# neverorfrog/vehicle-control

Hardware: AMD Instinct MI355X
Metric: MPC solves/sec (batched, N=20) (higher is better)
Workload: dtype f64; 1 GPU; C2 kinematic-bicycle LTV-MPC, B=1024 per GPU, N=20, fp64; batch_per_gpu=1024, global_batch=1024, horizon=20, parallelism=dp1 (independent shards)

## Files before the change

vehicle-control_amd/csrc/kin_ltv.hip:

```cpp
#include <hip/hip_runtime.h>

#include <cstdint>

#include "vc_kernels.hpp"
#include "vc_models.hpp"
#include "vcmpc.h"

#ifndef KIN_NU_TOL
#define KIN_NU_TOL 1e-10
#endif
#ifndef KIN_EARLY_F
#define KIN_EARLY_F 100.0
#endif
#ifndef KIN_EARLY_ROUNDS
#define KIN_EARLY_ROUNDS 2
#endif
#ifndef KIN_TAPIA_F
#define KIN_TAPIA_F 1.02
#endif
#ifndef KIN_DUAL_TOL
#define KIN_DUAL_TOL 1e-12
#endif
#ifndef KIN_AL_RHO
#define KIN_AL_RHO 1e1
#endif
#ifndef KIN_DOT_CH
#define KIN_DOT_CH 8
#endif
#ifndef KIN_UPDATE
#define KIN_UPDATE 1
#endif
#ifndef KIN_RSQ_HALLEY
#define KIN_RSQ_HALLEY 1
#endif
#ifndef KIN_STAT_CHECK
#define KIN_STAT_CHECK 0
#endif
#ifndef KIN_STEP_F
#define KIN_STEP_F 0.99
#endif
#ifndef KIN_SOLVE_CH
#define KIN_SOLVE_CH 8
#endif
#ifndef KIN_PANEL_CH
#define KIN_PANEL_CH 6
#endif

namespace vc {
namespace {

__device__ __forceinline__ double lane_bcast(double v, int src) {
  const int lo = __builtin_amdgcn_readlane(__double2loint(v), src);
  const int hi = __builtin_amdgcn_readlane(__double2hiint(v), src);
  return __hiloint2double(hi, lo);
}
__device__ int amdgcn_writelane(int v, int lane, int old) __asm("llvm.amdgcn.writelane.i32");
__device__ __forceinline__ double lane_put(double old, double v, int dst) {
  const int lo = amdgcn_writelane(__double2loint(v), dst, __double2loint(old));
  const int hi = amdgcn_writelane(__double2hiint(v), dst, __double2hiint(old));
  return __hiloint2double(hi, lo);
}
template <int K>
__device__ __forceinline__ double dpp_row_shr(double v, double ident) {
  const int lo = __builtin_amdgcn_update_dpp(__double2loint(ident), __double2loint(v), 0x110 + K, 0xf, 0xf, false);
  const int hi = __builtin_amdgcn_update_dpp(__double2hiint(ident), __double2hiint(v), 0x110 + K, 0xf, 0xf, false);
  return __hiloint2double(hi, lo);
}
template <typename Op>
__device__ __forceinline__ double wave_reduce(double v, double ident, Op op) {
  v = op(v, dpp_row_shr<1>(v, ident));
  v = op(v, dpp_row_shr<2>(v, ident));
  v = op(v, dpp_row_shr<4>(v, ident));
  v = op(v, dpp_row_shr<8>(v, ident));
  return op(op(lane_bcast(v, 15), lane_bcast(v, 31)), op(lane_bcast(v, 47), lane_bcast(v, 63)));
}
__device__ __forceinline__ double wave_sum(double v) {
  return wave_reduce(v, 0.0, [](double a, double b) { return a + b; });
}
__device__ __forceinline__ double wave_max(double v) {
  return wave_reduce(v, -__builtin_inf(), [](double a, double b) { return fmax(a, b); });
}
__device__ __forceinline__ double wave_min(double v) {
  return wave_reduce(v, __builtin_inf(), [](double a, double b) { return fmin(a, b); });
}
__device__ __forceinline__ void wave_sync() {
  asm volatile("" ::: "memory");
  __builtin_amdgcn_wave_barrier();
  asm volatile("" ::: "memory");
}
__device__ __forceinline__ void fence() { __builtin_amdgcn_sched_barrier(0); }
__device__ __forceinline__ int lane_opaque(int lane) {
  asm volatile("" : "+v"(lane));
  return lane;
}
__device__ __forceinline__ void no_hoist() { asm volatile("" ::: "memory"); }

using lds_cdouble = const __attribute__((address_space(3))) double;
__device__ __forceinline__ lds_cdouble* lds_opaque(const double* p) {
  uint32_t a = (uint32_t)(uintptr_t)(lds_cdouble*)p;
  asm volatile("" : "+v"(a));
  return (lds_cdouble*)(uintptr_t)a;
}

#ifdef VC_TIMING
#define VC_TSTAMP(var) \
  fence();              \
  const uint64_t var = __builtin_amdgcn_s_memtime(); \
  fence();
#define VC_TACC(slot, t0) \
  {                      \
    fence();             \
    tacc[slot] += __builtin_amdgcn_s_memtime() - (t0); \
    fence();             \
  }
#else
#define VC_TSTAMP(var)
#define VC_TACC(slot, t0)
#endif
enum { T_SWEEP = 0, T_SETUP, T_RESID, T_BUILD, T_CHOL, T_SOLVE, T_UPDATE, T_POLISH, T_OUT, T_S2, T_S3, T_S4, T_PAL, T_PPASS, T_NUPD, T_UCYC, T_NDROP, T_CFAIL, T_CRM, T_CADD, T_R0CHG, T_NSLOT };


template <int N>
struct Dims {
  static constexpr int n = 2 * N;
  static constexpr int NC = 2 * (N - 1);
  static constexpr int LD = n + 1;
  static_assert(n <= 64 && N >= 2, "one wavefront per problem needs 2 <= N <= 32");
};

template <int n>
__host__ __device__ constexpr int lc_base(int k) {
  static_assert(n % 2 == 0, "even n");
  return k * (n - 1) - k * (k - 1) / 2 + (k + 1) / 2;
}
template <int n>
__host__ __device__ constexpr int lc_start(int k) {
  return lc_base<n>(k) + k;
}

template <int N>
struct Smem {
  using D = Dims<N>;
  static constexpr int LC_DUMMY = lc_start<D::n>(D::n);
  static constexpr int LC_ZERO = LC_DUMMY + 1;
  double G[D::NC + 3][D::LD];
  double H[D::n + 1][D::LD];
  alignas(16) double Lc[LC_ZERO + 1];
  alignas(16) double zrow[48];
  double xb[N + 1][KIN_NX + 1];
  double jac[N + 1][9];
  double ub[D::n];
  double kap[N], ds[N];
  union {
    struct {
      double vz[64];
      double vc[64];
    };
    alignas(16) double tb2[128];
  };
  double dinv[64];
};

template <int N>
__host__ __device__ constexpr int crow_stage(int r) {
  return r < N - 1 ? r + 1 : r - (N - 1) + 1;
}

template <int LEN, int SA, int SB, int CH = KIN_DOT_CH>
__device__ __forceinline__ double lds_dot(lds_cdouble* a, lds_cdouble* b) {
  constexpr int NCH = (LEN + CH - 1) / CH;
  double ca[2][CH], cb[2][CH];
  auto fetch = [&](int c, int buf) {
#pragma unroll
    for (int q = 0; q < CH; ++q) {
      const int i = c * CH + q;
      ca[buf][q] = (i < LEN) ? a[i * SA] : 0.0;
      cb[buf][q] = (i < LEN) ? b[i * SB] : 0.0;
    }
  };
  double a0 = 0.0, a1 = 0.0;
  fetch(0, 0);
#pragma unroll
  for (int c = 0; c < NCH; ++c) {
    if (c + 1 < NCH) fetch(c + 1, (c + 1) & 1);
    fence();
#pragma unroll
    for (int q = 0; q < CH; q += 2) {
      a0 += ca[c & 1][q] * cb[c & 1][q];
      a1 += ca[c & 1][q + 1] * cb[c & 1][q + 1];
    }
  }
  fence();
  return a0 + a1;
}

template <int N>
__device__ double grow_dot(const Smem<N>& s, int lane) {
  constexpr int NC = Dims<N>::NC;
  const int r = lane < NC ? lane : 0;
  const double a = lds_dot<2 * (N - 1), 1, 1>(lds_opaque(&s.G[r][0]), lds_opaque(&s.vz[0]));
  return lane < NC ? a : 0.0;
}

template <int N>
__device__ double gt_dot(const Smem<N>& s, int lane) {
  constexpr int n = Dims<N>::n, NC = Dims<N>::NC, LD = Dims<N>::LD;
  const int j = lane < n ? lane : 0;
  const double a = lds_dot<NC, LD, 1>(lds_opaque(&s.G[0][j]), lds_opaque(&s.vc[0]));
  return lane < n ? a : 0.0;
}


template <int N>
__device__ double h_dot(const Smem<N>& s, int lane) {
  constexpr int n = Dims<N>::n;
  const int j = lane < n ? lane : 0;
  return lds_dot<n, 1, 1>(lds_opaque(&s.H[j][0]), lds_opaque(&s.vz[0]));
}

__device__ __forceinline__ void kin_sincos(double x, double& sn, double& cs) {
  const double n = __builtin_rint(x * 6.36619772367581382433e-01);
  const double y = fma(-n, 6.07710050650619224932e-11, fma(-n, 1.57079632673412561417e+00, x));
  const double z = y * y;
  const double rs = fma(z, fma(z, fma(z, fma(z, 1.58969099521155010221e-10, -2.50507602534068634195e-08),
                                      2.75573137070700676789e-06), -1.98412698298579493134e-04),
                        8.33333333332248946124e-03);
  const double sk = fma(z * y, fma(z, rs, -1.66666666666666324348e-01), y);
  const double rc = z * fma(z, fma(z, fma(z, fma(z, fma(z, -1.13596475577881948265e-11, 2.08757232129817482790e-09),
                                                  -2.75573143513906633035e-07), 2.48015872894767294178e-05),
                                   -1.38888888888741095749e-03), 4.16666666666666019037e-02);
  const double hz = 0.5 * z, w = 1.0 - hz;
  const double ck = w + (((1.0 - w) - hz) + z * rc);
  const int q = int(n) & 3;
  const double a = (q & 1) ? ck : sk, b = (q & 1) ? sk : ck;
  sn = (q & 2) ? -a : a;
  cs = ((q + 1) & 2) ? -b : b;
}

__device__ __forceinline__ double rsq_nr(double d) {
  double inv = __builtin_amdgcn_rsq(d);
#if KIN_RSQ_HALLEY
  const double e = fma(-d, inv * inv, 1.0);
  return fma(inv * e, fma(0.375, e, 0.5), inv);
#else
  inv = inv * (1.5 - 0.5 * d * inv * inv);
  inv = inv * (1.5 - 0.5 * d * inv * inv);
  return inv;
#endif
}

template <int N>
__device__ __forceinline__ void store_rows(const double (&Mr)[Dims<N>::n], Smem<N>& s, int lane) {
}

template <int N>
__device__ double chol_solve(const double (&Lr)[Dims<N>::n], const Smem<N>& s, double b, int lane) {
  constexpr int n = Dims<N>::n;
  constexpr int CH = KIN_SOLVE_CH;
  static_assert(n % CH == 0, "backward prefetch chunks");
  const int row = lane < n ? lane : 0;
  lds_cdouble* col = lds_opaque(&s.Lc[lc_base<n>(row)]);
  const double dj = s.dinv[row];
  double acc = b;
#pragma unroll
  for (int k = 0; k < n; ++k) acc -= Lr[k] * lane_bcast(acc * dj, k);
  acc *= dj;
  double x = 0.0;
  double lk[2][CH];
  lds_cdouble* zero = lds_opaque(&s.zrow[0]);
  auto fetch = [&](int c, int buf) {
    lds_cdouble* src = row < n - 1 - c * CH ? col : zero;
#pragma unroll
    for (int q = 0; q < CH; ++q) lk[buf][q] = src[n - 1 - c * CH - q];
  };
  fetch(0, 0);
#pragma unroll
  for (int c = 0; c < n / CH; ++c) {
    if (c + 1 < n / CH) fetch(c + 1, (c + 1) & 1);
    fence();
#pragma unroll
    for (int q = 0; q < CH; ++q) {
      const int k = n - 1 - c * CH - q;
      const double xk = lane_bcast(acc * dj, k);
      x = lane_put(x, xk, k);
      acc -= lk[c & 1][q] * xk;
    }
    fence();
  }
  return x;
}

enum { ROWS_G = 0, ROWS_E = 1 };
template <int N, int KIND>
__host__ __device__ constexpr int row_extent(int r) {
  if (KIND == ROWS_G) return r < Dims<N>::NC ? 2 * crow_stage<N>(r) : 0;
  return r < N ? 2 * (r + 1) : (r < N + 2 ? 2 * N : 0);
}
template <int N, int KIND>
__host__ __device__ constexpr int gram_rows() {
  return KIND == ROWS_G ? Dims<N>::NC : N + 2;
}
template <int N, int KIND>
__host__ __device__ constexpr bool kstep_hits(int ks, int I) {
  for (int q = 0; q < 4; ++q)
    if (row_extent<N, KIND>(4 * ks + q) > 16 * I) return true;
  return false;
}

using d4 = __attribute__((ext_vector_type(4))) double;
using d2 = __attribute__((ext_vector_type(2))) double;
template <int N>
struct Tiles {
  static constexpr int n = Dims<N>::n, NB = (n + 15) / 16, NT = NB * (NB + 1) / 2, BLD = 16 * NB + 2;
  static constexpr int count(bool full) { return full ? NB * NB : NT; }
};

template <int N, int KIND, bool FULL>
__device__ __forceinline__ void gram_mfma(d4 (&acc)[Tiles<N>::count(FULL)], const double* rows, const double* w,
                                          int lane) {
  constexpr int n = Dims<N>::n, LD = Dims<N>::LD, NB = Tiles<N>::NB;
  constexpr int KS = (gram_rows<N, KIND>() + 3) / 4;
  lane = lane_opaque(lane);
  const int lr = lane >> 4, lc = lane & 15;
  lds_cdouble* R = lds_opaque(rows);
  lds_cdouble* W = lds_opaque(w);
  double gk[KS][NB], wk[KS];
#pragma unroll
  for (int ks = 0; ks < KS; ++ks) {
    const int r = 4 * ks + lr;
    wk[ks] = W[r];
#pragma unroll
    for (int J = 0; J < NB; ++J) {
      const int c = 16 * J + lc;
      gk[ks][J] = R[r * LD + (c < n ? c : n)];
    }
  }
  fence();
#pragma unroll
  for (int ks = 0; ks < KS; ++ks) {
#pragma unroll
    for (int I = 0, t = 0; I < NB; ++I) {
      const double a = wk[ks] * gk[ks][I];
#pragma unroll
      for (int J = 0; J < (FULL ? NB : I + 1); ++J, ++t)
        if (kstep_hits<N, KIND>(ks, I > J ? I : J))
          acc[t] = __builtin_amdgcn_mfma_f64_16x16x4f64(a, gk[ks][J], acc[t], 0, 0, 0);
    }
  }
}

template <int N, bool FULL>
__device__ __forceinline__ void tiles_to_rows(double (&Mr)[Dims<N>::n], const d4 (&acc)[Tiles<N>::count(FULL)],
                                              Smem<N>& s, int lane) {
  constexpr int n = Dims<N>::n, NB = Tiles<N>::NB, BLD = Tiles<N>::BLD;
  static_assert(16 * BLD <= Smem<N>::LC_DUMMY, "transpose buffer must fit the factor storage");
  static_assert(16 * NB <= 48, "zero row length");
  lane = lane_opaque(lane);
  const int lr = lane >> 4, lc = lane & 15;
  double* buf = &s.Lc[0];
  const int myI = lane >> 4;
#pragma unroll
  for (int I = 0, t0 = 0; I < NB; ++I, t0 += FULL ? NB : I) {
    wave_sync();
#pragma unroll
    for (int J = 0; J < (FULL ? NB : I + 1); ++J) {
#pragma unroll
      for (int q = 0; q < 4; ++q) buf[(lr + 4 * q) * BLD + 16 * J + lc] = acc[t0 + J][q];
    }
    wave_sync();
    using lds_cd2 = const __attribute__((address_space(3))) d2;
    lds_cd2* brow = (lds_cd2*)lds_opaque(myI == I ? &buf[lc * BLD] : &s.zrow[0]);
#pragma unroll
    for (int i = 0; i < n; i += 2) {
      const int iend = FULL ? n : 16 * (I + 1);
      if (i < iend) {
        const d2 p = brow[i / 2];
        if (I == 0) { Mr[i] = p.x; Mr[i + 1] = p.y; }
        else { Mr[i] += p.x; Mr[i + 1] += p.y; }
      } else if (I == 0) {
        Mr[i] = 0.0;
        Mr[i + 1] = 0.0;
      }
    }
  }
  wave_sync();
}

template <int N>
__device__ __forceinline__ void build_normal_acc(d4 (&acc)[Tiles<N>::NT], Smem<N>& s, double wb, double hjj, int lane) {
  constexpr int n = Dims<N>::n, LD = Dims<N>::LD, NB = Tiles<N>::NB;
  static_assert(4 * ((Dims<N>::NC + 3) / 4) <= Dims<N>::NC + 2, "G zero rows cover the last k-step");
  lane = lane_opaque(lane);
  const int lr = lane >> 4, lc = lane & 15;
  const int jd = lane < n ? lane : n;
  s.H[jd][jd] = hjj + wb;
  wave_sync();
  {
    lds_cdouble* H = lds_opaque(&s.H[0][0]);
#pragma unroll
    for (int I = 0, t = 0; I < NB; ++I) {
#pragma unroll
      for (int J = 0; J <= I; ++J, ++t) {
        const int c = 16 * J + lc < n ? 16 * J + lc : n;
#pragma unroll
        for (int q = 0; q < 4; ++q) {
          const int r0 = 16 * I + 4 * q;
          acc[t][q] = r0 < n ? H[(r0 + lr) * LD + c] : 0.0;
        }
      }
    }
  }
  s.H[jd][jd] = hjj;
  gram_mfma<N, ROWS_G, false>(acc, &s.G[0][0], &s.vc[0], lane);
}

template <int N>
__device__ __forceinline__ void build_normal_mfma(double (&Mr)[Dims<N>::n], Smem<N>& s, double wb, double hjj,
                                                  int lane) {
  d4 acc[Tiles<N>::NT];
  build_normal_acc<N>(acc, s, wb, hjj, lane);
  tiles_to_rows<N, false>(Mr, acc, s, lane);
}

template <int N>
__device__ bool factor_blocked(double (&Mr)[Dims<N>::n], d4 (&acc)[Tiles<N>::NT], Smem<N>& s, int lane) {
  constexpr int n = Dims<N>::n, NB = Tiles<N>::NB;
  constexpr int DUMMY = Smem<N>::LC_DUMMY;
  static_assert(NB == 3 && n > 32 && n <= 40, "three panels, the last one at most 8 wide");
  static_assert(lc_start<n>(16) + 16 * 18 <= DUMMY, "panel 0/1 transpose buffer inside the factor storage");
  static_assert((lc_start<n>(16) & 1) == 0, "16-byte aligned transpose buffer");
  lane = lane_opaque(lane);
  const int lr = lane >> 4, lc = lane & 15, myI = lane >> 4;
  bool ok = true;
  double pa, pb, pc, pi1, pl21, pi2;
  auto part = [&](int p, int k) {
    if (p == 0) {
      pa = lane_bcast(Mr[k], k);
      pb = lane_bcast(Mr[k], k + 1);
      pc = lane_bcast(Mr[k + 1], k + 1);
      pi1 = rsq_nr(pa);
    } else if (p == 1) {
      pl21 = pb * pi1;
      const double d2 = fma(-pl21, pl21, pc);
      pi2 = rsq_nr(d2);
      ok = ok && (pa > 0.0) && (d2 > 0.0);
    } else {
      const double x = Mr[k] * pi1;
      const double y = fma(-x, pl21, Mr[k + 1]) * pi2;
      Mr[k] = x;
      Mr[k + 1] = y;
      s.Lc[lane >= k && lane < n ? lc_base<n>(k) + lane : DUMMY] = x;
      s.Lc[lane >= k + 1 && lane < n ? lc_base<n>(k + 1) + lane : DUMMY] = y;
      s.dinv[k] = pi1;
      s.dinv[k + 1] = pi2;
    }
  };
  using lds_cd2 = const __attribute__((address_space(3))) d2;
#pragma unroll
  for (int p = 0; p < NB; ++p) {
    const int c0 = 16 * p, c1 = (16 * p + 16 < n) ? 16 * p + 16 : n, W = c1 - c0;
    double* tb = p < 2 ? &s.Lc[lc_start<n>(16)] : &s.tb2[0];
    const int TS = p < 2 ? 18 : 10;
#pragma unroll
    for (int i = c0; i < c1; ++i) Mr[i] = 0.0;
#pragma unroll
    for (int I = p; I < NB; ++I) {
      const int t = I * (I + 1) / 2 + p;
      wave_sync();
#pragma unroll
      for (int q = 0; q < 4; ++q) {
        const int r = lr + 4 * q;
        if (4 * q < W)
          tb[(lc < W ? r * TS + lc : 8 * TS + lc)] = acc[t][q];
      }
      wave_sync();
      lds_cd2* src = (lds_cd2*)lds_opaque(myI == I && lc < W ? &tb[lc * TS] : &s.zrow[0]);
#pragma unroll
      for (int i = 0; i < W; i += 2) {
        const d2 v = src[i / 2];
        Mr[c0 + i] += v.x;
        Mr[c0 + i + 1] += v.y;
      }
    }
    wave_sync();
    part(0, c0);
    part(1, c0);
    part(2, c0);
#pragma unroll
    for (int k = c0; k + 2 < c1; k += 2) {
      wave_sync();
      fence();
      const double x = Mr[k], y = Mr[k + 1];
      Mr[k] = lane > k ? x : 0.0;
      Mr[k + 1] = lane > k + 1 ? y : 0.0;
      const double* cA = &s.Lc[lc_base<n>(k)];
      const double* cB = &s.Lc[lc_base<n>(k + 1)];
      constexpr int CH = KIN_PANEL_CH;
      const int J0 = k + 2, NCH = (c1 - J0 + CH - 1) / CH;
      double u0[2][CH], u1[2][CH];
      auto load = [&](int ch, int buf) {
#pragma unroll
        for (int q = 0; q < CH; ++q) {
          const int j = J0 + ch * CH + q;
          u0[buf][q] = j < c1 ? cA[j] : 0.0;
          u1[buf][q] = j < c1 ? cB[j] : 0.0;
        }
      };
      load(0, 0);
#pragma unroll
      for (int ch = 0; ch < NCH; ++ch) {
        if (ch + 1 < NCH) load(ch + 1, (ch + 1) & 1);
        fence();
#pragma unroll
        for (int q = 0; q < CH; ++q) {
          const int j = J0 + ch * CH + q;
          if (j < c1) Mr[j] = fma(-y, u1[ch & 1][q], fma(-x, u0[ch & 1][q], Mr[j]));
        }
        if (ch >= 1 && ch <= 3) part(ch - 1, k + 2);
        fence();
      }
#pragma unroll
      for (int pp = NCH - 1; pp < 3; ++pp) {
        part(pp < 0 ? 0 : pp, k + 2);
        fence();
      }
    }
    Mr[c1 - 2] = lane > c1 - 2 ? Mr[c1 - 2] : 0.0;
    Mr[c1 - 1] = lane > c1 - 1 ? Mr[c1 - 1] : 0.0;
    wave_sync();
    if (p + 1 < NB) {
      lds_cdouble* Lc = lds_opaque(&s.Lc[0]);
      lds_cdouble* Z = lds_opaque(&s.zrow[0]);
#pragma unroll
      for (int ks = 0; ks < W / 4; ++ks) {
        const int kk = c0 + 4 * ks + lr;
        double op[NB];
#pragma unroll
        for (int I = p + 1; I < NB; ++I) {
          const int jj = 16 * I + lc;
          op[I] = jj < n ? Lc[lc_base<n>(kk) + jj] : Z[0];
        }
#pragma unroll
        for (int I = p + 1; I < NB; ++I) {
#pragma unroll
          for (int J = p + 1; J <= I; ++J) {
            const int t = I * (I + 1) / 2 + J;
            acc[t] = __builtin_amdgcn_mfma_f64_16x16x4f64(-op[I], op[J], acc[t], 0, 0, 0);
          }
        }
      }
    }
  }
  store_rows<N>(Mr, s, lane);
  wave_sync();
  return ok;
}

__device__ __forceinline__ double wave_prefix(double v, int lane) {
  v += dpp_row_shr<1>(v, 0.0);
  v += dpp_row_shr<2>(v, 0.0);
  v += dpp_row_shr<4>(v, 0.0);
  v += dpp_row_shr<8>(v, 0.0);
  const double r0 = lane_bcast(v, 15), r1 = lane_bcast(v, 31), r2 = lane_bcast(v, 47);
  return v + (lane >= 16 ? r0 : 0.0) + (lane >= 32 ? r1 : 0.0) + (lane >= 48 ? r2 : 0.0);
}

template <int N>
__device__ bool factor_update(double (&Mr)[Dims<N>::n], Smem<N>& s, int upd, int j, bool fixed, double sqrho,
                              int lane) {
  constexpr int n = Dims<N>::n;
  constexpr int DUMMY = Smem<N>::LC_DUMMY, ZERO = Smem<N>::LC_ZERO;
  lane = lane_opaque(lane);
  const int row = lane < n ? lane : 0;
  auto below = [&](int k, int other) { return lane > k && lane < n ? lc_base<n>(k) + lane : other; };
  double z;
  if (upd == 1) {
    z = s.Lc[below(j, ZERO)];
    wave_sync();
    s.Lc[below(j, DUMMY)] = 0.0;
    s.Lc[lane < j ? lc_base<n>(lane) + j : DUMMY] = 0.0;
    s.Lc[lc_start<n>(j)] = 1.0;
    s.dinv[j] = 1.0;
  } else {
    z = (lane < n && !fixed) ? sqrho * s.G[j][lane < n ? lane : n] : 0.0;
  }
  wave_sync();
  {
    lds_cdouble* L = lds_opaque(&s.Lc[0]);
#pragma unroll
    for (int k = 0; k < n; ++k) Mr[k] = L[below(k, ZERO)];
  }
  const double dj = s.dinv[row];
  double acc = z;
#pragma unroll
  for (int k = 0; k < n; ++k) acc -= Mr[k] * lane_bcast(acc * dj, k);
  const double y = lane < n ? acc * dj : 0.0;
  const double t = 1.0 + wave_prefix(y * y, lane);
  const double sk = sqrt(t / (t - y * y)), ck = y / t;
  const bool ok = __ballot(!(sk > 0.5 && sk < 1e150)) == 0ull;
  wave_sync();
  if (lane < n) {
    s.Lc[lc_start<n>(row)] *= sk;
    s.dinv[row] = dj / sk;
  }
  s.tb2[2 * lane] = ck;
  s.tb2[2 * lane + 1] = sk;
  wave_sync();
  {
    using lds_cd2 = const __attribute__((address_space(3))) d2;
    lds_cd2* cs = (lds_cd2*)lds_opaque(&s.tb2[0]);
    double w = z;
#pragma unroll
    for (int k = 0; k < n - 1; ++k) {
      const double yk = lane_bcast(y, k);
      const d2 c = cs[k];
      w = lane_put(w, 0.0, k);
      const double l = Mr[k];
      w = fma(-yk, l, w);
      Mr[k] = fma(c.x, w, l) * c.y;
    }
  }
#pragma unroll
  for (int k = 0; k < n - 1; ++k) s.Lc[below(k, DUMMY)] = Mr[k];
  wave_sync();
  return ok;
}

struct Side {
  double lo, hi, slo, shi, llo, lhi;
  bool hasLo, hasHi;
};

}

template <int N>
__global__ __launch_bounds__(64) void kin_ltv_kernel(KinLtvArgs A) {
  using D = Dims<N>;
  constexpr int n = D::n, NC = D::NC;
  __shared__ Smem<N> s;
  const int lane = threadIdx.x;
  const int b = xcd_problem(blockIdx.x, A.B);
  if (b >= A.B) return;
  const vc_kin_mpc& W = A.w;

  if (lane < n) s.ub[lane] = A.ubar[(size_t)b * n + lane];
  if (lane < N) {
    s.kap[lane] = A.kappa[(size_t)b * N + lane];
    s.ds[lane] = A.ds[(size_t)b * N + lane];
  }
  if (lane < KIN_NX) s.xb[0][lane] = A.x0[(size_t)b * KIN_NX + lane];
  for (int i = lane; i < 2 * D::LD; i += 64) (&s.G[NC][0])[i] = 0.0;
  if (lane < 48) s.zrow[lane] = 0.0;
  if (lane == 0) s.Lc[Smem<N>::LC_ZERO] = 0.0;
  wave_sync();

#ifdef VC_TIMING
  uint64_t tacc[T_NSLOT] = {};
#endif
  VC_TSTAMP(t_sweep0)
  constexpr int LD = Dims<N>::LD;
  double* E = &s.H[0][0];
  bool finite = true;
  {
    double x[KIN_NX];
#pragma unroll
    for (int i = 0; i < KIN_NX; ++i) x[i] = s.xb[0][i];
#pragma unroll 1
    for (int k = 0; k < N; ++k) {
      const double u2[2] = {s.ub[2 * k], s.ub[2 * k + 1]};
      const double h = s.ds[k];
      double f[KIN_NX];
      {
        double sn, cs;
        kin_sincos((lane & 1) ? x[1] : x[4], sn, cs);
        const double se = lane_bcast(sn, 0), ce = lane_bcast(cs, 0);
        const double sd = lane_bcast(sn, 1), cd = lane_bcast(cs, 1);
        const double kap = s.kap[k];
        const double rho = 1.0 - x[3] * kap;
        const int r4 = lane & 3;
        const double num = r4 == 0 ? se : (r4 == 1 ? sd : rho);
        const double den = r4 == 0 ? ce : (r4 == 1 ? cd * A.L : (r4 == 2 ? ce : x[0] * ce));
        const double quo = num * rcp_nr(den);
        const double te = lane_bcast(quo, 0), tdl = lane_bcast(quo, 1);
        const double rc = lane_bcast(quo, 2), q = lane_bcast(quo, 3);
        f[0] = q * u2[0];
        f[1] = q * u2[1];
        f[2] = 1.0;
        f[3] = rho * te;
        f[4] = tdl * rc - kap;
        f[5] = q;
      }
      double mine = 0.0;
#pragma unroll
      for (int i = 0; i < KIN_NX; ++i) {
        x[i] += h * f[i];
        finite = finite && isfinite(x[i]);
        mine = (i == lane) ? x[i] : mine;
      }
      s.xb[k + 1][lane < KIN_NX ? lane : KIN_NX] = mine;
      const double ey = x[3];
      double cw, lin;
      if (k + 1 < N) {
        const double hs = s.ds[k + 1];
        cw = W.w_dev * hs;
        lin = W.w_dev * hs * ey;
        if (ey < W.ey_min) { cw += W.w_b * hs; lin += W.w_b * hs * (ey - W.ey_min); }
        if (ey > W.ey_max) { cw += W.w_b * hs; lin += W.w_b * hs * (ey - W.ey_max); }
      } else {
        cw = W.w_ey;
        lin = W.w_ey * ey;
      }
      s.vc[k] = 2.0 * cw;
      s.vz[k] = 2.0 * lin;
    }
  }
  wave_sync();
  VC_TACC(T_SWEEP, t_sweep0)
  VC_TSTAMP(t_s20)
  {
    const int k = lane < N ? lane : 0;
    double xk[KIN_NX];
#pragma unroll
    for (int i = 0; i < KIN_NX; ++i) xk[i] = s.xb[k][i];
    const KinJac J = kin_spatial_jac(xk, s.kap[k], A.L);
    double* jr = s.jac[lane < N ? lane : N];
    jr[0] = J.q; jr[1] = J.qv; jr[2] = J.qey; jr[3] = J.qep;
    jr[4] = J.J33; jr[5] = J.J34; jr[6] = J.J41; jr[7] = J.J43; jr[8] = J.J44;
    if (A.obs.n > 0 && lane >= 1 && lane < N) {
      double p, q;
      obstacle_ey_model<double>(A.obs, xk[2], xk[3], W.w_obs * s.ds[k], p, q);
      s.vc[k - 1] += q;
      s.vz[k - 1] += p;
    }
  }
  wave_sync();
  VC_TACC(T_S2, t_s20)
  VC_TSTAMP(t_s30)
  double gj = 0.0;
  double cv = 0, cd = 0, cey = 0, cep = 0, ct = 0;
  {
    const int jcol = lane < n ? lane : n;
    double jn[9], hn, an, wn;
    auto fetch = [&](int k) {
#pragma unroll
      for (int q = 0; q < 9; ++q) jn[q] = s.jac[k][q];
      hn = s.ds[k]; an = s.ub[2 * k]; wn = s.ub[2 * k + 1];
    };
    fetch(0);
#pragma unroll 1
    for (int k = 0; k < N; ++k) {
      double J[9];
#pragma unroll
      for (int q = 0; q < 9; ++q) J[q] = jn[q];
      const double h = hn, a = an, w = wn;
      const double lin2 = s.vz[k];
      if (k + 1 < N) fetch(k + 1);
      const double dq = J[1] * cv + J[2] * cey + J[3] * cep;
      const double ncv = cv + h * a * dq + (lane == 2 * k ? h * J[0] : 0.0);
      const double ncd = cd + h * w * dq + (lane == 2 * k + 1 ? h * J[0] : 0.0);
      const double ncey = cey + h * (J[4] * cey + J[5] * cep);
      const double ncep = cep + h * (J[6] * cd + J[7] * cey + J[8] * cep);
      ct += h * dq;
      cv = ncv; cd = ncd; cey = ncey; cep = ncep;
      const bool has = k + 1 <= N - 1;
      s.G[has ? k : NC + 2][jcol] = cv;
      s.G[has ? (N - 1) + k : NC + 2][jcol] = cd;
      E[k * LD + jcol] = cey;
      gj += lin2 * cey;
    }
    E[N * LD + jcol] = cv;
    E[(N + 1) * LD + jcol] = cep;
  }
  wave_sync();
  VC_TACC(T_S3, t_s30)
  VC_TSTAMP(t_s40)
  double Hr[n];
  double hjj;
  {
    const double vN = s.xb[N][0];
    const double cwv = (vN >= W.v_max) ? W.w_v : 0.0;
    gj += 2.0 * cwv * (vN - W.v_max) * cv;
    gj += 2.0 * W.w_epsi * s.xb[N][4] * cep;
    gj += W.w_time * ct;
    if (lane < 4) s.vc[N + lane] = lane == 0 ? 2.0 * cwv : (lane == 1 ? 2.0 * W.w_epsi : 0.0);
    for (int i = lane; i < 2 * LD; i += 64) E[(N + 2) * LD + i] = 0.0;
    wave_sync();
    d4 acc[Tiles<N>::count(true)];
#pragma unroll
    for (int t = 0; t < Tiles<N>::count(true); ++t) acc[t] = d4{0.0, 0.0, 0.0, 0.0};
    gram_mfma<N, ROWS_E, true>(acc, E, &s.vc[0], lane);
    tiles_to_rows<N, true>(Hr, acc, s, lane);
  }
  const int kq = lane >> 1;
  double dself = 2.0 * A.qp.prox, dm2 = 0.0, dp2 = 0.0;
  if (lane < n) {
    if (lane & 1) {
      dself += 2.0 * W.w_w;
      gj += 2.0 * W.w_w * s.ub[lane];
    } else {
      if (kq >= 1) {
        dself += 2.0 * W.w_a; dm2 = -2.0 * W.w_a;
        gj += 2.0 * W.w_a * (s.ub[lane] - s.ub[lane - 2]);
      }
      if (kq <= N - 2) {
        dself += 2.0 * W.w_a; dp2 = -2.0 * W.w_a;
        gj -= 2.0 * W.w_a * (s.ub[lane + 2] - s.ub[lane]);
      }
    }
  }
  gj = (lane < n) ? gj : 0.0;
  {
    const int j = lane < n ? lane : n;
#pragma unroll
    for (int i = 0; i < n; ++i) s.H[j][i] = Hr[i];
    s.H[j][n] = 0.0;
    s.H[j][j] += dself;
    s.H[j][j >= 2 ? j - 2 : j] += dm2;
    s.H[j][j + 2 < n ? j + 2 : j] += dp2;
    hjj = lane < n ? s.H[j][j] : 0.0;
  }
  wave_sync();
  if (A.mode == 1) {
    if (lane < n) {
#pragma unroll
      for (int i = 0; i < n; ++i) A.H_out[((size_t)b * n + lane) * n + i] = s.H[lane][i];
      A.g_out[(size_t)b * n + lane] = gj;
    }
    return;
  }

  VC_TACC(T_S4, t_s40)
  VC_TSTAMP(t_setup0)
  Side bx, cs;
  {
    const bool isw = lane & 1;
    const double u = (lane < n) ? s.ub[lane] : 0.0;
    bx.lo = (isw ? W.w_min : W.a_min) - u;
    bx.hi = (isw ? W.w_max : W.a_max) - u;
    const double tr = isw ? A.qp.trust_w : A.qp.trust_a;
    if (tr > 0.0) {
      bx.lo = fmax(bx.lo, -tr);
      bx.hi = fmin(bx.hi, tr);
    }
    bx.hasLo = bx.hasHi = (lane < n);
    const int st = crow_stage<N>(lane < NC ? lane : 0);
    if (lane < N - 1) {
      cs.lo = W.v_min - s.xb[st][0];
      cs.hi = 0.0;
      cs.hasLo = true; cs.hasHi = false;
    } else if (lane < NC) {
      cs.lo = W.delta_min - s.xb[st][1];
      cs.hi = W.delta_max - s.xb[st][1];
      cs.hasLo = cs.hasHi = true;
    } else {
      cs.lo = cs.hi = 0.0;
      cs.hasLo = cs.hasHi = false;
    }
  }
  const double mtot = double(4 * N + 3 * (N - 1));
  double scale, hdiag_max;
  {
    double m = fabs(gj);
    if (bx.hasLo) m = fmax(m, fabs(bx.lo));
    if (bx.hasHi) m = fmax(m, fabs(bx.hi));
    if (cs.hasLo) m = fmax(m, fabs(cs.lo));
    if (cs.hasHi) m = fmax(m, fabs(cs.hi));
    scale = 1.0 + wave_max(m);
    hdiag_max = fmax(wave_max(hjj), 1.0);
  }
  double z = 0.0;
  bx.slo = bx.hasLo ? fmax(-bx.lo, 1.0) : 1.0;
  bx.shi = bx.hasHi ? fmax(bx.hi, 1.0) : 1.0;
  bx.llo = bx.hasLo ? 1.0 : 0.0;
  bx.lhi = bx.hasHi ? 1.0 : 0.0;
  cs.slo = cs.hasLo ? fmax(-cs.lo, 1.0) : 1.0;
  cs.shi = cs.hasHi ? fmax(cs.hi, 1.0) : 1.0;
  cs.llo = cs.hasLo ? 1.0 : 0.0;
  cs.lhi = cs.hasHi ? 1.0 : 0.0;

  VC_TACC(T_SETUP, t_setup0)
  const int max_iter = A.qp.max_iter;
  const double tol = A.qp.tol * scale;
  int it = 0;
  bool converged = false, chol_fail = false, near = false;
  double last_res = 0.0, last_mu = 0.0;
  double Mr[n];
  double rd = 0.0, rlo_b = 0.0, rhi_b = 0.0, rlo_c = 0.0, rhi_c = 0.0;
  auto true_residuals = [&]() {
    wave_sync();
    s.vz[lane] = (lane < n) ? z : 0.0;
    s.vc[lane] = (lane < NC) ? (cs.lhi - cs.llo) : 0.0;
    wave_sync();
    const double yc = grow_dot<N>(s, lane);
    rd = (lane < n) ? (h_dot<N>(s, lane) + gj + (bx.lhi - bx.llo) + gt_dot<N>(s, lane)) : 0.0;
    rlo_b = bx.hasLo ? (z - bx.lo - bx.slo) : 0.0;
    rhi_b = bx.hasHi ? (bx.hi - z - bx.shi) : 0.0;
    rlo_c = cs.hasLo ? (yc - cs.lo - cs.slo) : 0.0;
    rhi_c = cs.hasHi ? (cs.hi - yc - cs.shi) : 0.0;
  };
  auto max_residual = [&]() {
    return wave_max(fmax(fmax(fabs(rd), fmax(fabs(rlo_b), fabs(rhi_b))), fmax(fabs(rlo_c), fabs(rhi_c))));
  };
  int tapb = 0;
  const double tol_early = KIN_EARLY_F > 0.0 ? fmax(tol, KIN_EARLY_F * tol) : tol;
  int e_set = 0;
#ifdef VC_TIMING
  uint64_t e_fmask = 0;
  bool e_row = false, e_have = false;
#endif
  double tol_cur = tol_early;
  bool polished = false, pchol_fail = false;
  int rounds = 0;
#pragma unroll 1
  for (;;) {
  if (finite) {
#pragma unroll 1
    for (;;) {
      no_hoist();
      VC_TSTAMP(t_res0)
      if (it == 0) true_residuals();
      const double mu = wave_sum(bx.slo * bx.llo + bx.shi * bx.lhi + cs.slo * cs.llo + cs.shi * cs.lhi) / mtot;
      double res = max_residual();
      if (it > 0 && res <= tol_cur && mu <= tol_cur) {
        true_residuals();
        res = max_residual();
      }
      converged = res <= tol_cur && mu <= tol_cur;
      last_res = res;
      last_mu = mu;
      if (converged || it >= max_iter || !isfinite(res) || !isfinite(mu)) break;
      ++it;
      const double wlo_b = bx.hasLo ? bx.llo / bx.slo : 0.0;
      const double whi_b = bx.hasHi ? bx.lhi / bx.shi : 0.0;
      const double wlo_c = cs.hasLo ? cs.llo / cs.slo : 0.0;
      const double whi_c = cs.hasHi ? cs.lhi / cs.shi : 0.0;
      wave_sync();
      s.vc[lane] = (lane < NC) ? wlo_c + whi_c : 0.0;
      wave_sync();
      VC_TACC(T_RESID, t_res0)
      VC_TSTAMP(t_build0)
      d4 nacc[Tiles<N>::NT];
      build_normal_acc<N>(nacc, s, wlo_b + whi_b, hjj, lane);
      VC_TACC(T_BUILD, t_build0)
      VC_TSTAMP(t_chol0)
      const bool chol_ok = factor_blocked<N>(Mr, nacc, s, lane);
      VC_TACC(T_CHOL, t_chol0)
      if (!chol_ok) {
        chol_fail = true;
        near = res <= 1e-6 * scale && mu <= tol;
        break;
      }
      const double islo_b = bx.hasLo ? rcp_nr(bx.slo) : 0.0, ishi_b = bx.hasHi ? rcp_nr(bx.shi) : 0.0;
      const double islo_c = cs.hasLo ? rcp_nr(cs.slo) : 0.0, ishi_c = cs.hasHi ? rcp_nr(cs.shi) : 0.0;
      const double illo_b = bx.hasLo ? rcp_nr(bx.llo) : 0.0, ilhi_b = bx.hasHi ? rcp_nr(bx.lhi) : 0.0;
      const double illo_c = cs.hasLo ? rcp_nr(cs.llo) : 0.0, ilhi_c = cs.hasHi ? rcp_nr(cs.lhi) : 0.0;
      double sm = 0.0, pp1 = 0.0, pp2 = 0.0, pp3 = 0.0, pp4 = 0.0;
#pragma unroll 1
      for (int pass = 0; pass < 2; ++pass) {
        no_hoist();
        const double rclo_b = bx.slo * bx.llo + pp1 - sm, rchi_b = bx.shi * bx.lhi + pp2 - sm;
        const double rclo_c = cs.slo * cs.llo + pp3 - sm, rchi_c = cs.shi * cs.lhi + pp4 - sm;
        const double eb = (bx.hasHi ? (-rchi_b * ishi_b - whi_b * rhi_b) : 0.0) +
                          (bx.hasLo ? (rclo_b * islo_b + wlo_b * rlo_b) : 0.0);
        const double ec = (cs.hasHi ? (-rchi_c * ishi_c - whi_c * rhi_c) : 0.0) +
                          (cs.hasLo ? (rclo_c * islo_c + wlo_c * rlo_c) : 0.0);
        wave_sync();
        s.vc[lane] = (lane < NC) ? ec : 0.0;
        wave_sync();
        const double rhs = (lane < n) ? (-rd - eb - gt_dot<N>(s, lane)) : 0.0;
        VC_TSTAMP(t_sol0)
        const double dz = chol_solve<N>(Mr, s, rhs, lane);
        VC_TACC(T_SOLVE, t_sol0)
        wave_sync();
        s.vz[lane] = (lane < n) ? dz : 0.0;
        wave_sync();
        const double dyc = grow_dot<N>(s, lane);
        const double d1 = bx.hasLo ? dz + rlo_b : 0.0;
        const double d2 = bx.hasLo ? (-rclo_b * islo_b - wlo_b * (dz + rlo_b)) : 0.0;
        const double d3 = bx.hasHi ? rhi_b - dz : 0.0;
        const double d4 = bx.hasHi ? (-rchi_b * ishi_b - whi_b * (rhi_b - dz)) : 0.0;
        const double e1 = cs.hasLo ? dyc + rlo_c : 0.0;
        const double e2 = cs.hasLo ? (-rclo_c * islo_c - wlo_c * (dyc + rlo_c)) : 0.0;
        const double e3 = cs.hasHi ? rhi_c - dyc : 0.0;
        const double e4 = cs.hasHi ? (-rchi_c * ishi_c - whi_c * (rhi_c - dyc)) : 0.0;
        const double tmax = wave_max(fmax(fmax(fmax(-d1 * islo_b, -d2 * illo_b), fmax(-d3 * ishi_b, -d4 * ilhi_b)),
                                          fmax(fmax(-e1 * islo_c, -e2 * illo_c), fmax(-e3 * ishi_c, -e4 * ilhi_c))));
        const double amax = 1.0 / fmax(1.0, tmax);
        if (pass == 0) {
          const double mua = wave_sum((bx.slo + amax * d1) * (bx.llo + amax * d2) +
                                      (bx.shi + amax * d3) * (bx.lhi + amax * d4) +
                                      (cs.slo + amax * e1) * (cs.llo + amax * e2) +
                                      (cs.shi + amax * e3) * (cs.lhi + amax * e4)) / mtot;
          const double sr = mua / mu;
          sm = sr * sr * sr * mu;
          pp1 = d1 * d2; pp2 = d3 * d4; pp3 = e1 * e2; pp4 = e3 * e4;
        } else {
          const double al = KIN_STEP_F * amax;
          {
            auto tap = [&](double dl, double il, double dsv, double is) -> int {
              const double lr = fma(al * dl, il, 1.0), sr = fma(al * dsv, is, 1.0);
              return lr > KIN_TAPIA_F * sr ? 1 : (sr > KIN_TAPIA_F * lr ? 2 : 0);
            };
            tapb = tap(d2, illo_b, d1, islo_b) | (tap(d4, ilhi_b, d3, ishi_b) << 2) |
                   (tap(e2, illo_c, e1, islo_c) << 4) | (tap(e4, ilhi_c, e3, ishi_c) << 6);
          }
          z = (lane < n) ? z + al * dz : z;
          bx.slo += al * d1; bx.llo += al * d2; bx.shi += al * d3; bx.lhi += al * d4;
          cs.slo += al * e1; cs.llo += al * e2; cs.shi += al * e3; cs.lhi += al * e4;
          const double om = 1.0 - al;
          rd *= om; rlo_b *= om; rhi_b *= om; rlo_c *= om; rhi_c *= om;
        }
      }
    }
  }

  VC_TSTAMP(t_pol0)
  if ((converged || near) && A.qp.polish > 0) {
    constexpr double AL_RHO = KIN_AL_RHO;
    constexpr int AL_MAX = 16;
    const double ptol = 1e-9 * scale, dtol = KIN_DUAL_TOL * scale;
    auto guess = [&](bool has, double l, double sv, int t) { return has && (t == 1 || (t == 0 && l > sv)); };
    bool alo_b = guess(bx.hasLo, bx.llo, bx.slo, tapb & 3);
    bool ahi_b = guess(bx.hasHi, bx.lhi, bx.shi, (tapb >> 2) & 3);
    bool alo_c = guess(cs.hasLo, cs.llo, cs.slo, (tapb >> 4) & 3);
    bool ahi_c = guess(cs.hasHi, cs.lhi, cs.shi, (tapb >> 6) & 3);
    auto pack = [&]() { return int(alo_b) | (int(ahi_b) << 1) | (int(alo_c) << 2) | (int(ahi_c) << 3); };
    if (tol_cur <= tol && __ballot(e_set != 0 && pack() != (e_set & 15)) == 0ull && __ballot(e_set != 0) != 0ull) {
      const int t = e_set >> 4;
      alo_b = t & 1; ahi_b = (t >> 1) & 1; alo_c = (t >> 2) & 1; ahi_c = (t >> 3) & 1;
    }
    const int max_rounds = tol_cur > tol ? min(A.qp.polish, KIN_EARLY_ROUNDS) : A.qp.polish;
    double rho_k = 0.0;
    int upd = 0, upd_j = 0;
#pragma unroll 1
    for (int round = 0; round < max_rounds; ++round) {
      no_hoist();
      const int set0 = pack();
#ifdef VC_TIMING
      if (round == 0 && tol_cur <= tol && e_have) {
        const bool fx = (lane < n) && (alo_b || ahi_b);
        const uint64_t fm = __ballot(fx);
        const bool ract = (lane < NC) && (alo_c || ahi_c);
        tacc[T_CFAIL] = 1;
        tacc[T_CRM] = __builtin_popcountll(e_fmask & ~fm) + __builtin_popcountll(__ballot(e_row && !ract));
        tacc[T_CADD] = __builtin_popcountll(fm & ~e_fmask) + __builtin_popcountll(__ballot(ract && !e_row));
      }
#endif
      ++rounds;
      const bool fixed = (lane < n) && (alo_b || ahi_b);
      const double zfix = fixed ? (alo_b ? bx.lo : bx.hi) : 0.0;
      const uint64_t fmask = __ballot(fixed);
      const bool act = (lane < NC) && (alo_c || ahi_c);
      wave_sync();
      s.vz[lane] = (lane < n) ? zfix : 0.0;
      wave_sync();
      const double gfix = grow_dot<N>(s, lane);
      double gn2 = 0.0;
      {
        const int r = lane < NC ? lane : 0;
#pragma unroll 2
        for (int i = 0; i < 2 * (N - 1); ++i) {
          const double gi = ((fmask >> i) & 1ull) ? 0.0 : s.G[r][i];
          gn2 += gi * gi;
        }
      }
      const double rho_new = (act && gn2 > 1e-28) ? AL_RHO * hdiag_max / gn2 : 0.0;
      const double rho_c = (KIN_UPDATE && rho_k > 0.0 && rho_new > 0.0) ? rho_k : rho_new;
      const double bnd_c = act ? ((alo_c ? cs.lo : cs.hi) - gfix) : 0.0;
      const double base = (lane < n) ? -(gj + h_dot<N>(s, lane)) : 0.0;
      wave_sync();
      s.vc[lane] = rho_c;
      wave_sync();
      VC_TSTAMP(t_pf0)
      bool updated = false;
      if (KIN_UPDATE && upd != 0) {
        const bool same = __ballot(lane < NC && rho_c != rho_k && !(upd == 2 && lane == upd_j)) == 0ull;
        VC_TSTAMP(t_u0)
        if (same) updated = factor_update<N>(Mr, s, upd, upd_j, fixed, sqrt(lane_bcast(rho_c, upd_j)), lane);
#ifdef VC_TIMING
        if (updated) tacc[T_NUPD] += 1;
#endif
        VC_TACC(T_UCYC, t_u0)
      }
      rho_k = rho_c;
      if (!updated) {
        d4 pacc[Tiles<N>::NT];
        build_normal_acc<N>(pacc, s, 0.0, hjj, lane);
        const int pl = lane_opaque(lane), plr = pl >> 4, plc = pl & 15;
#pragma unroll
        for (int I = 0, t = 0; I < Tiles<N>::NB; ++I) {
#pragma unroll
          for (int J = 0; J <= I; ++J, ++t) {
            const int c = 16 * J + plc;
            const bool fc = (fmask >> c) & 1ull;
#pragma unroll
            for (int q = 0; q < 4; ++q) {
              const int r = 16 * I + plr + 4 * q;
              const bool fr = (fmask >> r) & 1ull;
              pacc[t][q] = (fr || fc) ? (r == c ? 1.0 : 0.0) : pacc[t][q];
            }
          }
        }
        if (!factor_blocked<N>(Mr, pacc, s, lane)) {
          pchol_fail = true;
          break;
        }
      }
      VC_TACC(T_UPDATE, t_pf0)
      VC_TSTAMP(t_pal0)
      double nu_c = (act && rho_c > 0.0) ? ((ahi_c ? cs.lhi : 0.0) - (alo_c ? cs.llo : 0.0)) : 0.0;

      const bool al_act = act && rho_c > 0.0;
      const double bnd_al = alo_c ? cs.lo : cs.hi;
      double zp = 0.0, emax = 0.0;
      {
        wave_sync();
        s.vc[lane] = (lane < NC) ? (nu_c - rho_c * bnd_c) : 0.0;
        wave_sync();
        const double rhs = (lane < n) ? (fixed ? zfix : (base - gt_dot<N>(s, lane))) : 0.0;
        zp = chol_solve<N>(Mr, s, rhs, lane);
        wave_sync();
        s.vz[lane] = (lane < n) ? zp : 0.0;
        wave_sync();
        const double yr = grow_dot<N>(s, lane);
        double rr = al_act ? (yr - bnd_al) : 0.0;
        const double ie = 1.0 / (1e-14 * scale), inu = KIN_NU_TOL > 0.0 ? 1.0 / (KIN_NU_TOL * scale) : 0.0;
        auto crit = [&](double r) { return wave_max(fmax(fabs(r) * ie, fabs(rho_c * r) * inu)); };
#ifdef VC_TIMING
        tacc[T_PPASS] += 1;
#endif
        if (crit(rr) > 1.0) {
          double pd = rho_c * rr;
          double rz = wave_sum(rr * pd);
#pragma unroll 1
          for (int it = 1; it < AL_MAX; ++it) {
            no_hoist();
            wave_sync();
            s.vc[lane] = (lane < NC) ? pd : 0.0;
            wave_sync();
            const double gtp = gt_dot<N>(s, lane);
            const double zq = chol_solve<N>(Mr, s, (lane < n && !fixed) ? gtp : 0.0, lane);
            wave_sync();
            s.vz[lane] = (lane < n) ? zq : 0.0;
            wave_sync();
            const double gq = grow_dot<N>(s, lane);
            const double q = al_act ? gq : 0.0;
            const double pq = wave_sum(pd * q);
#ifdef VC_TIMING
            tacc[T_PPASS] += 1;
#endif
            if (!(pq > 0.0)) break;
            const double al = rz / pq;
            nu_c = fma(al, pd, nu_c);
            zp = fma(-al, zq, zp);
            rr = fma(-al, q, rr);
            if (crit(rr) <= 1.0) break;
            const double zt = rho_c * rr;
            const double rzn = wave_sum(rr * zt);
            pd = fma(rzn / rz, pd, zt);
            rz = rzn;
          }
        }
      }
      VC_TACC(T_PAL, t_pal0)
      wave_sync();
      s.vz[lane] = (lane < n) ? zp : 0.0;
      s.vc[lane] = (lane < NC) ? nu_c : 0.0;
      wave_sync();
      const double grad = (lane < n) ? (h_dot<N>(s, lane) + gj + gt_dot<N>(s, lane)) : 0.0;
      const double ypc = grow_dot<N>(s, lane);
#if KIN_STAT_CHECK
      emax = wave_max(fmax(al_act ? fabs(ypc - bnd_al) : 0.0, (lane < n && !fixed) ? fabs(grad) : 0.0));
#else
      emax = wave_max(al_act ? fabs(ypc - bnd_al) : 0.0);
#endif
      const double dv_b = (lane < n) ? (ahi_b ? grad : (alo_b ? -grad : -1.0)) : -1.0;
      const double dv_c = (lane < NC) ? (ahi_c ? -nu_c : (alo_c ? nu_c : -1.0)) : -1.0;
      const double pv_b = (lane < n && !fixed) ? fmax(bx.lo - zp, zp - bx.hi) : -1.0;
      const double pv_c = (lane < NC && !(act && rho_c > 0.0))
                              ? fmax(cs.hasLo ? cs.lo - ypc : -1.0, cs.hasHi ? ypc - cs.hi : -1.0)
                              : -1.0;
      const double dmax = wave_max(fmax(dv_b, dv_c));
      const double pmax = wave_max(fmax(pv_b, pv_c));
      if (dmax <= dtol && pmax <= ptol) {
        if (emax <= ptol) {
          z = (lane < n) ? zp : z;
          polished = true;
        }
        break;
      }
      const bool dual = dmax > dtol;
      const double worst = dual ? dmax : pmax;
      const double vb = dual ? dv_b : pv_b, vcr = dual ? dv_c : pv_c;
      const uint64_t who = __ballot(fmax(vb, vcr) == worst);
      const int sel = __builtin_ffsll((long long)who) - 1;
      const bool sel_box = (__ballot(vb >= vcr) >> sel) & 1ull;
      upd = dual ? 0 : (sel_box ? 1 : 2);
      upd_j = sel;
#ifdef VC_TIMING
      if (dual) tacc[T_NDROP] += 1;
#endif
      if (lane == sel) {
        if (vb >= vcr) {
          if (dual) { alo_b = false; ahi_b = false; }
          else if (zp < bx.lo) alo_b = true;
          else ahi_b = true;
        } else {
          if (dual) { alo_c = false; ahi_c = false; }
          else if (ypc < cs.lo) alo_c = true;
          else ahi_c = true;
        }
      }
#ifdef VC_TIMING
      int r0code = 0;
      if (tol_cur > tol && round == 0) {
        int tside = 0;
        if (vb >= vcr) tside = (dual ? (ahi_b ? (tapb >> 2) : tapb) : (zp < bx.lo ? tapb : (tapb >> 2))) & 3;
        else tside = (dual ? (ahi_c ? (tapb >> 6) : (tapb >> 4)) : (ypc < cs.lo ? (tapb >> 4) : (tapb >> 6))) & 3;
        const int code = 1 + (dual ? 2 : (vb >= vcr ? 0 : 1)) + 3 * tside;
        r0code = __builtin_amdgcn_readlane(code, sel);
#ifdef VC_TIMING
        tacc[T_R0CHG] = (uint64_t)r0code;
#endif
      }
#endif
      if (tol_cur > tol) e_set = 256 | set0 | (pack() << 4);
#ifdef VC_TIMING
      if (tol_cur > tol) {
        e_fmask = fmask;
        e_row = rho_k > 0.0;
        e_have = true;
      }
#endif
    }
  }

  VC_TACC(T_POLISH, t_pol0)
  if (polished || !converged || chol_fail || tol_cur <= tol) break;
  tol_cur = tol;
  converged = false;
  pchol_fail = false;
  }
  VC_TSTAMP(t_out0)
  int32_t st;
  if (!finite) st = VC_NONFINITE;
  else if (polished || converged) st = VC_SOLVED;
  else st = VC_MAX_ITER;
  if (!finite) z = 0.0;
  wave_sync();
  if (lane < n) {
    s.vz[lane] = z;
    A.u_out[(size_t)b * n + lane] = s.ub[lane] + z;
  }
  wave_sync();
  if (lane < 2) A.u0[(size_t)b * 2 + lane] = s.ub[lane] + s.vz[lane];
  if (lane == 0) {
    A.status[b] = st;
    A.iters[b] = it;
    if (A.diag) {
#ifdef VC_TIMING
      constexpr size_t DS = 4 + T_NSLOT;
#else
      constexpr size_t DS = 4;
#endif
      A.diag[(size_t)b * DS + 0] = last_res / scale;
      A.diag[(size_t)b * DS + 1] = last_mu / scale;
      A.diag[(size_t)b * DS + 2] = double((chol_fail ? 1 : 0) | (converged ? 2 : 0) | (polished ? 4 : 0) |
                                          (pchol_fail ? 8 : 0));
      A.diag[(size_t)b * DS + 3] = double(rounds);
    }
  }
  double dx[KIN_NX] = {0, 0, 0, 0, 0, 0};
  double* xo = A.x_out + (size_t)b * (N + 1) * KIN_NX;
  if (lane < KIN_NX) xo[lane] = s.xb[0][lane];
#pragma unroll 1
  for (int k = 0; k < N; ++k) {
    const double q = s.jac[k][0], qv = s.jac[k][1], qey = s.jac[k][2], qep = s.jac[k][3];
    const double h = s.ds[k], a = s.ub[2 * k], w = s.ub[2 * k + 1];
    const double da = s.vz[2 * k], dw = s.vz[2 * k + 1];
    const double dq = qv * dx[0] + qey * dx[3] + qep * dx[4];
    double nx[KIN_NX];
    nx[0] = dx[0] + h * (a * dq + q * da);
    nx[1] = dx[1] + h * (w * dq + q * dw);
    nx[2] = dx[2];
    nx[3] = dx[3] + h * (s.jac[k][4] * dx[3] + s.jac[k][5] * dx[4]);
    nx[4] = dx[4] + h * (s.jac[k][6] * dx[1] + s.jac[k][7] * dx[3] + s.jac[k][8] * dx[4]);
    nx[5] = dx[5] + h * dq;
    double mine = 0.0;
#pragma unroll
    for (int i = 0; i < KIN_NX; ++i) {
      dx[i] = nx[i];
      if (i == lane) mine = nx[i];
    }
    if (lane < KIN_NX) xo[(k + 1) * KIN_NX + lane] = s.xb[k + 1][lane] + mine;
  }
  VC_TACC(T_OUT, t_out0)
#ifdef VC_TIMING
  if (A.diag && lane < T_NSLOT) {
    double v = 0.0;
#pragma unroll
    for (int i = 0; i < T_NSLOT; ++i) v = (i == lane) ? double(tacc[i]) : v;
    A.diag[(size_t)b * (4 + T_NSLOT) + 4 + lane] = v;
  }
#endif
}

size_t kin_ltv_smem_bytes(int N) {
  switch (N) {
    case 20: return sizeof(Smem<20>);
    default: return 0;
  }
}

hipError_t launch_kin_ltv(const KinLtvArgs& a, int N, hipStream_t stream) {
  if (a.B <= 0) return hipSuccess;
  switch (N) {
    case 20:
      hipLaunchKernelGGL(kin_ltv_kernel<20>, dim3(a.B), dim3(64), 0, stream, a);
      return hipGetLastError();
    default:
      return hipErrorInvalidValue;
  }
}

}
```

Before: 5.165 million solves/s.

## Parallelize forward sweep weights and output trajectory rollout across lanes

The nominal-state sweep now keeps only the state update in the serial loop, with lane 0 writing states. The tracking-cost weights for every stage are then computed in parallel by one lane per stage, and the finiteness check is done once after the loop. The final linearized trajectory reconstruction replaces a 20-step serial loop on all lanes with a short serial recurrence for only the lateral states, followed by a lane-parallel evaluation using shuffles and a wave prefix sum, then a coalesced write of x_out. It also adds timing slots for the step phase and the whole kernel. The risk is numerical drift from the reordered sums and the fma contractions, plus extra syncs; the change also assumes the solution vector layout matches grow_dot and the tb2 slot mapping.

New measurement: 5.305 million solves/s, median of 6. 1.03x the previous value.

```diff
diff --git a/vehicle-control_amd/csrc/kin_ltv.hip b/vehicle-control_amd/csrc/kin_ltv.hip
--- a/vehicle-control_amd/csrc/kin_ltv.hip
+++ b/vehicle-control_amd/csrc/kin_ltv.hip
@@ -117,7 +117,7 @@
 #define VC_TSTAMP(var)
 #define VC_TACC(slot, t0)
 #endif
-enum { T_SWEEP = 0, T_SETUP, T_RESID, T_BUILD, T_CHOL, T_SOLVE, T_UPDATE, T_POLISH, T_OUT, T_S2, T_S3, T_S4, T_PAL, T_PPASS, T_NUPD, T_UCYC, T_NDROP, T_CFAIL, T_CRM, T_CADD, T_R0CHG, T_NSLOT };
+enum { T_SWEEP = 0, T_SETUP, T_RESID, T_BUILD, T_CHOL, T_SOLVE, T_UPDATE, T_POLISH, T_OUT, T_S2, T_S3, T_S4, T_PAL, T_PPASS, T_NUPD, T_UCYC, T_NDROP, T_CFAIL, T_CRM, T_CADD, T_R0CHG, T_STEP, T_TOTAL, T_NSLOT };
 
 
 template <int N>
@@ -642,6 +642,10 @@
   const int b = xcd_problem(blockIdx.x, A.B);
   if (b >= A.B) return;
   const vc_kin_mpc& W = A.w;
+#ifdef VC_TIMING
+  uint64_t tacc[T_NSLOT] = {};
+#endif
+  VC_TSTAMP(t_all0)
 
   if (lane < n) s.ub[lane] = A.ubar[(size_t)b * n + lane];
   if (lane < N) {
@@ -654,9 +658,6 @@
   if (lane == 0) s.Lc[Smem<N>::LC_ZERO] = 0.0;
   wave_sync();
 
-#ifdef VC_TIMING
-  uint64_t tacc[T_NSLOT] = {};
-#endif
   VC_TSTAMP(t_sweep0)
   constexpr int LD = Dims<N>::LD;
   double* E = &s.H[0][0];
@@ -690,29 +691,35 @@
         f[4] = tdl * rc - kap;
         f[5] = q;
       }
-      double mine = 0.0;
-#pragma unroll
-      for (int i = 0; i < KIN_NX; ++i) {
-        x[i] += h * f[i];
-        finite = finite && isfinite(x[i]);
-        mine = (i == lane) ? x[i] : mine;
-      }
-      s.xb[k + 1][lane < KIN_NX ? lane : KIN_NX] = mine;
-      const double ey = x[3];
-      double cw, lin;
-      if (k + 1 < N) {
-        const double hs = s.ds[k + 1];
-        cw = W.w_dev * hs;
-        lin = W.w_dev * hs * ey;
-        if (ey < W.ey_min) { cw += W.w_b * hs; lin += W.w_b * hs * (ey - W.ey_min); }
-        if (ey > W.ey_max) { cw += W.w_b * hs; lin += W.w_b * hs * (ey - W.ey_max); }
-      } else {
-        cw = W.w_ey;
-        lin = W.w_ey * ey;
-      }
-      s.vc[k] = 2.0 * cw;
-      s.vz[k] = 2.0 * lin;
-    }
+#pragma unroll
+      for (int i = 0; i < KIN_NX; ++i) x[i] += h * f[i];
+      if (lane == 0) {
+#pragma unroll
+        for (int i = 0; i < KIN_NX; ++i) s.xb[k + 1][i] = x[i];
+      }
+    }
+#pragma unroll
+    for (int i = 0; i < KIN_NX; ++i) finite = finite && isfinite(x[i]);
+  }
+  wave_sync();
+  if (lane < N) {
+    const double ey = s.xb[lane + 1][3];
+    double cw, lin;
+    if (lane + 1 < N) {
+      const double hs = s.ds[lane + 1];
+      const double td = W.w_dev * hs;
+      double tb = W.w_b * hs;
+      asm volatile("" : "+v"(tb));
+      cw = td;
+      lin = ey * td;
+      if (ey < W.ey_min) { cw = __builtin_fma(W.w_dev, hs, tb); lin = __builtin_fma(ey - W.ey_min, tb, lin); }
+      if (ey > W.ey_max) { cw = cw + tb; lin = __builtin_fma(ey - W.ey_max, tb, lin); }
+    } else {
+      cw = W.w_ey;
+      lin = W.w_ey * ey;
+    }
+    s.vc[lane] = 2.0 * cw;
+    s.vz[lane] = 2.0 * lin;
   }
   wave_sync();
   VC_TACC(T_SWEEP, t_sweep0)
@@ -950,6 +957,10 @@
         near = res <= 1e-6 * scale && mu <= tol;
         break;
       }
+#ifdef VC_TIMING
+      const uint64_t t_sol_before = tacc[T_SOLVE];
+#endif
+      VC_TSTAMP(t_step0)
       const double islo_b = bx.hasLo ? rcp_nr(bx.slo) : 0.0, ishi_b = bx.hasHi ? rcp_nr(bx.shi) : 0.0;
       const double islo_c = cs.hasLo ? rcp_nr(cs.slo) : 0.0, ishi_c = cs.hasHi ? rcp_nr(cs.shi) : 0.0;
       const double illo_b = bx.hasLo ? rcp_nr(bx.llo) : 0.0, ilhi_b = bx.hasHi ? rcp_nr(bx.lhi) : 0.0;
@@ -1011,6 +1022,10 @@
           rd *= om; rlo_b *= om; rhi_b *= om; rlo_c *= om; rhi_c *= om;
         }
       }
+      VC_TACC(T_STEP, t_step0)
+#ifdef VC_TIMING
+      tacc[T_STEP] -= tacc[T_SOLVE] - t_sol_before;
+#endif
     }
   }
 
@@ -1270,31 +1285,48 @@
       A.diag[(size_t)b * DS + 3] = double(rounds);
     }
   }
-  double dx[KIN_NX] = {0, 0, 0, 0, 0, 0};
-  double* xo = A.x_out + (size_t)b * (N + 1) * KIN_NX;
-  if (lane < KIN_NX) xo[lane] = s.xb[0][lane];
-#pragma unroll 1
-  for (int k = 0; k < N; ++k) {
+  {
+    const double y = grow_dot<N>(s, lane);
+    const int slot = lane < N - 1 ? 64 + lane + 1
+                                  : (lane < NC ? n + (lane - (N - 1)) + 1 : (lane == NC ? 64 : (lane == NC + 1 ? n : 127)));
+    wave_sync();
+    s.tb2[slot] = y;
+    wave_sync();
+    double ey = 0.0, ep = 0.0, eyk = 0.0, epk = 0.0;
+#pragma unroll 4
+    for (int k = 0; k < N; ++k) {
+      const double h = s.ds[k], dd = s.vz[n + k];
+      eyk = lane_put(eyk, ey, k);
+      epk = lane_put(epk, ep, k);
+      const double ney = ey + h * (s.jac[k][4] * ey + s.jac[k][5] * ep);
+      const double nep = ep + h * (s.jac[k][6] * dd + s.jac[k][7] * ey + s.jac[k][8] * ep);
+      ey = ney; ep = nep;
+    }
+    eyk = lane_put(eyk, ey, N);
+    epk = lane_put(epk, ep, N);
+    const double eyn = __shfl_down(eyk, 1), epn = __shfl_down(epk, 1);
+    const int k = lane < N ? lane : 0;
     const double q = s.jac[k][0], qv = s.jac[k][1], qey = s.jac[k][2], qep = s.jac[k][3];
     const double h = s.ds[k], a = s.ub[2 * k], w = s.ub[2 * k + 1];
     const double da = s.vz[2 * k], dw = s.vz[2 * k + 1];
-    const double dq = qv * dx[0] + qey * dx[3] + qep * dx[4];
-    double nx[KIN_NX];
-    nx[0] = dx[0] + h * (a * dq + q * da);
-    nx[1] = dx[1] + h * (w * dq + q * dw);
-    nx[2] = dx[2];
-    nx[3] = dx[3] + h * (s.jac[k][4] * dx[3] + s.jac[k][5] * dx[4]);
-    nx[4] = dx[4] + h * (s.jac[k][6] * dx[1] + s.jac[k][7] * dx[3] + s.jac[k][8] * dx[4]);
-    nx[5] = dx[5] + h * dq;
-    double mine = 0.0;
-#pragma unroll
-    for (int i = 0; i < KIN_NX; ++i) {
-      dx[i] = nx[i];
-      if (i == lane) mine = nx[i];
-    }
-    if (lane < KIN_NX) xo[(k + 1) * KIN_NX + lane] = s.xb[k + 1][lane] + mine;
+    const double dv = s.vc[k], dd = s.vz[n + k];
+    const double dq = qv * dv + qey * eyk + qep * epk;
+    const double dt = wave_prefix(lane < N ? h * dq : 0.0, lane);
+    wave_sync();
+    if (lane < N) {
+      double* xr = s.xb[k + 1];
+      xr[0] += dv + h * (a * dq + q * da);
+      xr[1] += dd + h * (w * dq + q * dw);
+      xr[3] += eyn;
+      xr[4] += epn;
+      xr[5] += dt;
+    }
+    wave_sync();
+    double* xo = A.x_out + (size_t)b * (N + 1) * KIN_NX;
+    for (int i = lane; i < (N + 1) * KIN_NX; i += 64) xo[i] = s.xb[i / KIN_NX][i % KIN_NX];
   }
   VC_TACC(T_OUT, t_out0)
+  VC_TACC(T_TOTAL, t_all0)
 #ifdef VC_TIMING
   if (A.diag && lane < T_NSLOT) {
     double v = 0.0;
```
